# Weepingchestnut/SAVSR

Measured on AMD Instinct MI355X. Metric: HR Mpixels/sec (Vid4-shape x4, 7-frame window), higher is better.
Workload: dtype f32 (bf16x3 split products, fp32 accumulate)

## Files before the change

### savsr_amd/csrc/conv_wy.hip

```cpp
#include "conv_common.hpp"

#include <type_traits>

#ifndef WY_STAMPS
#define WY_STAMPS 0
#endif
#ifndef WY_VALU
#define WY_VALU 6
#endif
#ifndef WY_FAST_EPILOGUE
#define WY_FAST_EPILOGUE 1
#endif
#ifndef WY_BUF
#define WY_BUF 1
#endif

namespace savsr {

namespace wy {
constexpr int TH = 16, TW = 32, NTHR = 512, COT = 64;
[[maybe_unused]] constexpr int IC = TW + 2;
#ifndef WY_ICP
#define WY_ICP 36
#endif
constexpr int ICP = WY_ICP;
constexpr int V_PLANE = 2 * ICP;
constexpr int V_WAVE = 2 * 2 * 2 * V_PLANE;
constexpr int W_HALF = 6 * 2 * 2 * 64;
constexpr int W_PHASE = 2 * W_HALF;
constexpr int EPS = 36;
constexpr int LDS_UNITS = 8 * V_WAVE + 2 * W_HALF;
constexpr size_t LDS_BYTES = 16ull * LDS_UNITS + 4ull * 8 * 32 * EPS;
static_assert(LDS_BYTES <= 160 * 1024, "LDS budget");
}

__device__ __attribute__((aligned(16))) const float g_wy_zero16[4] = {0.f, 0.f, 0.f, 0.f};

#if WY_STAMPS
__device__ long long g_wy_stamps[256 * 8 * 8];
#define WY_KSEC(i) (WY_STAMPS == 2 ? 0 : (i))
#define WY_MARK(i) do { const long long t_now = (long long)__builtin_amdgcn_s_memtime(); wy_sec[i] += t_now - wy_prev; wy_prev = t_now; } while (0)
#if WY_STAMPS == 2
#define WY_EMARK(i) WY_MARK(i)
#endif
#else
#define WY_KSEC(i) (i)
#define WY_MARK(i) do { } while (0)
#endif

typedef float f32x2 __attribute__((ext_vector_type(2)));
typedef __bf16 bf16x2 __attribute__((ext_vector_type(2)));
__device__ __forceinline__ void wy_split_store(const f32x4& v, bf16x4* hi_dst, bf16x4* lo_dst) {
    typedef unsigned u32x2 __attribute__((ext_vector_type(2)));
    const f32x2 a[2] = {{v[0], v[1]}, {v[2], v[3]}};
    u32x2 hi, lo;
#pragma unroll
    for (int p = 0; p < 2; ++p) hi[p] = __builtin_bit_cast(unsigned, __builtin_convertvector(a[p], bf16x2));
    asm("" : "+v"(hi[0]), "+v"(hi[1]));
#pragma unroll
    for (int p = 0; p < 2; ++p) {
        const f32x2 back = {__builtin_bit_cast(float, hi[p] << 16), __builtin_bit_cast(float, hi[p] & 0xffff0000u)};
        const f32x2 rest = {a[p][0] - back[0], a[p][1] - back[1]};
        lo[p] = __builtin_bit_cast(unsigned, __builtin_convertvector(rest, bf16x2));
    }
    *hi_dst = __builtin_bit_cast(bf16x4, hi);
    *lo_dst = __builtin_bit_cast(bf16x4, lo);
}
__device__ __forceinline__ void wy_f16_store(const f32x4& v, bf16x4* hi_dst) {
    f16x4 h;
#pragma unroll
    for (int j = 0; j < 4; ++j) h[j] = (_Float16)v[j];
    *hi_dst = __builtin_bit_cast(bf16x4, h);
}

template <bool FAST, bool F16>
__global__ __launch_bounds__(512) void conv_wy_kernel(const MultiConvParams mp) {
    using namespace wy;
    constexpr int WPH = F16 ? W_PHASE / 2 : W_PHASE, WHF = F16 ? W_HALF / 2 : W_HALF;
    extern __shared__ __attribute__((aligned(16))) unsigned char smem_raw[];
    bf16x8* smem = reinterpret_cast<bf16x8*>(smem_raw);
    const int tid = threadIdx.x, lane = tid & 63, wave = tid >> 6, half = lane >> 5, px = lane & 31;
    const int wave_s = __builtin_amdgcn_readfirstlane(wave);
    const int tiles_per_cob = mp.wy_tiles;
    const int total = mp.nconv * mp.ncob * tiles_per_cob;
    const int H = mp.h, W = mp.w;

    struct TileInfo { int conv, cob, x0, y0, tx, ty, strip; };
    auto decode = [&](int tile) {
        const int cc = (int)((unsigned)tile / (unsigned)tiles_per_cob), rem = tile - cc * tiles_per_cob;
        const bool strip = rem >= mp.wy_full;
        const int tyf = (int)((unsigned)rem / (unsigned)mp.ntx);
        const int l2 = strip ? mp.wy_strip_l2 : 3;
        const int ty = strip ? mp.nty - 1 : tyf;
        const int tx = strip ? (rem - mp.wy_full) << (3 - l2) : rem - tyf * mp.ntx;
        const int wx = tx + (wave_s >> l2);
        TileInfo ti;
        ti.conv = (int)((unsigned)cc / (unsigned)mp.ncob);
        ti.cob = cc - ti.conv * mp.ncob;
        ti.x0 = (wx < mp.ntx ? wx : tx) * TW;
        ti.y0 = wx < mp.ntx ? ty * TH - 2 * ((wave_s >> l2) << l2) : mp.nty * TH;
        ti.tx = tx;
        ti.ty = ty;
        ti.strip = strip ? 1 : 0;
        return ti;
    };

    f32x4 d[2][4], dx;
#if !WY_BUF
    int st_pxb[2], st_pxt;
    constexpr int INVALID = -(1 << 30);
#endif
    const float* st_base = nullptr;
    const bf16x8* st_w = nullptr;
    int st_pix = 0, st_cb = 0, st_src = 0, st_conv = 0, st_row0 = 0;
    const int q4 = lane & 3;
#if WY_BUF
    constexpr unsigned OOB = 0x80000000u;
    unsigned st_vcol[2], st_vtail;
    int st_x0 = 0;
    auto stage_cols = [&]() {
#pragma unroll
        for (int r = 0; r < 2; ++r) {
            const int x = st_x0 - 1 + (lane >> 2) + 16 * r;
            const unsigned v = (unsigned)(x * st_pix + 4 * q4) * 4u;
            st_vcol[r] = (unsigned)x < (unsigned)W ? v : OOB;
        }
        const int x = st_x0 - 1 + 32 + ((lane & 7) >> 2), rr = (lane >> 3) & 3, row = st_row0 + rr;
        const unsigned vt = (unsigned)((rr * W + x) * st_pix + 4 * q4) * 4u;
        const bool okt = (lane < 32) & ((unsigned)x < (unsigned)W) & ((unsigned)row < (unsigned)H);
        st_vtail = okt ? vt : OOB;
    };
#endif
#if WY_BUF
    auto uni = [](int v) { return __builtin_amdgcn_readfirstlane(v); };
    auto uni_ptr = [](const float* q) {
        const unsigned long long a = (unsigned long long)(uintptr_t)q;
        const unsigned lo = (unsigned)__builtin_amdgcn_readfirstlane((int)(unsigned)a), hi = (unsigned)__builtin_amdgcn_readfirstlane((int)(unsigned)(a >> 32));
        return (const float*)(uintptr_t)(((unsigned long long)hi << 32) | lo);
    };
#else
    auto uni = [](int v) { return v; };
    auto uni_ptr = [](const float* q) { return q; };
#endif
    auto stage_begin_tile = [&](const TileInfo& ti) {
        st_conv = ti.conv;
        st_src = 0;
        st_cb = 0;
        st_base = uni_ptr(mp.c[ti.conv].src[0]);
        st_pix = uni(mp.c[ti.conv].src_pix[0]);
        st_w = reinterpret_cast<const bf16x8*>(mp.c[ti.conv].wimg) + (long long)ti.cob * mp.nchunk * WPH;
        st_row0 = uni(ti.y0 + 2 * wave_s - 1);
#if WY_BUF
        st_x0 = ti.x0;
        stage_cols();
#else
#pragma unroll
        for (int r = 0; r < 2; ++r) {
            const int x = ti.x0 - 1 + (lane >> 2) + 16 * r;
            st_pxb[r] = (x >= 0 && x < W) ? st_row0 * W + x : INVALID;
        }
        {
            const int x = ti.x0 - 1 + 32 + ((lane & 7) >> 2), row = st_row0 + ((lane >> 3) & 3);
            st_pxt = (lane < 32 && x >= 0 && x < W && row >= 0 && row < H) ? row * W + x : INVALID;
        }
#endif
    };
    auto stage_advance = [&]() {
        st_cb += 16;
        st_w += WPH;
        if (st_cb >= mp.src_ch) {
            st_cb = 0;
            ++st_src;
            st_base = uni_ptr(mp.c[st_conv].src[st_src]);
#if WY_BUF
            const int pix_new = uni(mp.c[st_conv].src_pix[st_src]);
            if (pix_new != st_pix) { st_pix = pix_new; stage_cols(); }
#else
            st_pix = mp.c[st_conv].src_pix[st_src];
#endif
        }
    };
    int st_tile = blockIdx.x, st_chunk = 0;
    auto stage_next = [&]() -> bool {
        if (st_chunk + 1 < mp.nchunk) { ++st_chunk; stage_advance(); return true; }
        if (st_tile + (int)gridDim.x >= total) return false;
        st_tile += gridDim.x;
        st_chunk = 0;
        stage_begin_tile(decode(st_tile));
        return true;
    };
#if WY_BUF
    typedef unsigned u32x4_t __attribute__((ext_vector_type(4)));
    auto row_rsrc = [&](int i, bool whole) {
        const int off = ((st_row0 + i) * W * st_pix + st_cb) * 4;
        const bool row_ok = whole || (st_row0 + i >= 0 && st_row0 + i < H);
        return __builtin_amdgcn_make_buffer_rsrc((void*)((const char*)st_base + off), (short)0, row_ok ? 0x7fffffff : 0, 0x00020000);
    };
    auto issue_row = [&](int r, int i) {
        d[r][i] = __builtin_bit_cast(f32x4, (u32x4_t)__builtin_amdgcn_raw_buffer_load_b128(row_rsrc(i, false), (int)st_vcol[r], 0, 0));
    };
    auto issue_d = [&](int r) {
#pragma unroll
        for (int i = 0; i < 4; ++i) issue_row(r, i);
    };
    auto issue_dx = [&]() { dx = __builtin_bit_cast(f32x4, (u32x4_t)__builtin_amdgcn_raw_buffer_load_b128(row_rsrc(0, true), (int)st_vtail, 0, 0)); };
#else
    auto load_at = [&](int pixel, bool ok) -> f32x4 {
        const SAVSR_GLOBAL float* src = ok ? (const SAVSR_GLOBAL float*)st_base + (pixel * st_pix + st_cb + 4 * q4)
                                           : (const SAVSR_GLOBAL float*)g_wy_zero16;
        return *(const SAVSR_GLOBAL f32x4*)src;
    };
    auto issue_row = [&](int r, int i) {
        const bool row_ok = st_row0 + i >= 0 && st_row0 + i < H;
        d[r][i] = load_at(st_pxb[r] + i * W, row_ok && st_pxb[r] != INVALID);
    };
    auto issue_d = [&](int r) {
#pragma unroll
        for (int i = 0; i < 4; ++i) issue_row(r, i);
    };
    auto issue_dx = [&]() { dx = load_at(st_pxt, st_pxt != INVALID); };
#endif
    bf16x8* vwave = smem + wave * V_WAVE;
    constexpr int PLANE_B = V_PLANE * 16;
    const unsigned vst0 = (unsigned)(wave * V_WAVE + (q4 >> 1) * ICP + (lane >> 2)) * 16u + (unsigned)(q4 & 1) * 8u;
    const unsigned vst_t = (unsigned)(wave * V_WAVE + (q4 >> 1) * ICP + 32 + ((lane & 7) >> 2)) * 16u + (unsigned)(q4 & 1) * 8u;
    auto vptr = [&](unsigned off) { return reinterpret_cast<bf16x4*>(smem_raw + off); };
    auto vstore = [&](const f32x4& v, unsigned off) {
        if constexpr (F16) wy_f16_store(v, vptr(off));
        else wy_split_store(v, vptr(off), vptr(off + PLANE_B));
    };
    auto store_pair = [&](int r, int hf, const f32x4& va, const f32x4& vb) {
        vstore(va, vst0 + (unsigned)(r * 256 + (hf * 2 + 0) * 2 * PLANE_B));
        vstore(vb, vst0 + (unsigned)(r * 256 + (hf * 2 + 1) * 2 * PLANE_B));
    };
    auto store_one = [&](int r, int hf, int vr, const f32x4& v) {
        vstore(v, vst0 + (unsigned)(r * 256 + (hf * 2 + vr) * 2 * PLANE_B));
    };
    auto store_v0 = [&](int r) { store_one(r, 0, 0, d[r][0] - d[r][2]); };
    auto store_v1 = [&](int r) {
        store_one(r, 0, 1, d[r][1] + d[r][2]);
        const f32x4 v2 = d[r][2] - d[r][1], v3 = d[r][1] - d[r][3];
        d[r][0] = v2;
        d[r][1] = v3;
    };
    auto store_v01 = [&](int r) { store_v0(r); store_v1(r); };
    auto store_v23 = [&](int r) { store_pair(r, 1, d[r][0], d[r][1]); };
    const int grp = (lane >> 3) & 3;
    auto tail_value = [&](int hf) -> f32x4 {
        const int partner = hf == 0 ? (grp == 0 ? lane ^ 16 : lane ^ 24) : (grp == 2 ? lane ^ 24 : lane ^ 16);
        f32x4 o;
#pragma unroll
        for (int j = 0; j < 4; ++j) o[j] = __shfl(dx[j], partner, 64);
        return (hf == 0 && grp == 1) ? dx + o : dx - o;
    };
    auto tail_store = [&](int hf, const f32x4& v) {
        const bool mine = lane < 32 && (hf == 0 ? grp < 2 : (grp == 2 || grp == 1));
        const int vr = hf == 0 ? grp : (grp == 2 ? 0 : 1);
        if (mine) {
            vstore(v, vst_t + (unsigned)((hf * 2 + vr) * 2 * PLANE_B));
        }
    };
    auto store_vt01 = [&]() {
        const f32x4 v01 = tail_value(0), v23 = tail_value(1);
        tail_store(0, v01);
        dx = v23;
    };
    auto store_vt23 = [&]() { tail_store(1, dx); };
    bf16x8* wlds = smem + 8 * V_WAVE;
    [[maybe_unused]] const unsigned lane16 = (unsigned)lane * 16u;
    auto issue_w = [&](int j, int hf) {
        const int piece = F16 ? j * 8 + wave_s : wave_s * 3 + j;
        if (F16 && piece >= 12) return;
        const unsigned dst = __builtin_amdgcn_readfirstlane((unsigned)(uintptr_t)(wlds + hf * W_HALF + piece * (F16 ? 128 : 64)));
        unsigned keep;
#if WY_BUF
        asm volatile("s_mov_b32 %0, m0\n\ts_mov_b32 m0, %3\n\ts_nop 0\n\tglobal_load_lds_dwordx4 %1, %2\n\ts_mov_b32 m0, %0"
                     : "=&s"(keep) : "v"(lane16), "s"(st_w + hf * WHF + piece * 64), "s"(dst) : "memory");
#else
        asm volatile("s_mov_b32 %0, m0\n\ts_mov_b32 m0, %2\n\ts_nop 0\n\tglobal_load_lds_dwordx4 %1, off\n\ts_mov_b32 m0, %0"
                     : "=&s"(keep) : "v"(st_w + hf * WHF + piece * 64 + lane), "s"(dst) : "memory");
#endif
    };

    struct FragA { bf16x8 ah, al; };
    struct FragB { bf16x8 bh, bl; };
    const bf16x8* vrd = vwave + half * ICP + px;
    const bf16x8* wrd = wlds + lane;
    auto load_b = [&](int hf, int s, FragB& fr) {
        const int vr = s / 3, kx = s - 3 * vr;
        fr.bh = vrd[((hf * 2 + vr) * 2 + 0) * V_PLANE + kx];
        if (!F16) fr.bl = vrd[((hf * 2 + vr) * 2 + 1) * V_PLANE + kx];
    };
    auto load_a = [&](int hf, int s, int t, FragA& fr) {
        fr.ah = wrd[hf * W_HALF + ((s * 2 + t) * 2 + 0) * 64];
        if (!F16) fr.al = wrd[hf * W_HALF + ((s * 2 + t) * 2 + 1) * 64];
    };

    int tile = blockIdx.x;
#if WY_STAMPS
    long long wy_sec[8] = {0, 0, 0, 0, 0, 0, 0, 0};
    long long wy_prev = (long long)__builtin_amdgcn_s_memtime();
    const long long wy_t0 = wy_prev;
#endif
    FragA fa[2];
    FragB fb[2];
    if (tile < total) {
        stage_begin_tile(decode(tile));
#pragma unroll
        for (int j = 0; j < 3; ++j) issue_w(j, 0);
        issue_d(0);
        issue_d(1);
        issue_dx();
        store_v01(0);
        store_v01(1);
        store_vt01();
    }
    asm volatile("s_waitcnt vmcnt(0)" ::: "memory");
    __syncthreads();
    if (tile < total) { load_b(0, 0, fb[0]); load_a(0, 0, 0, fa[0]); }

    for (; tile < total; tile += gridDim.x) {
        const TileInfo cur = decode(tile);
        const ConvParams& p = mp.c[cur.conv];
        const int cob = cur.cob, x0 = cur.x0, y0 = cur.y0;
        f32x16 acc[4][2];
#pragma unroll
        for (int pz = 0; pz < 4; ++pz)
#pragma unroll
            for (int t = 0; t < 2; ++t)
#pragma unroll
                for (int i = 0; i < 16; ++i) acc[pz][t][i] = 0.f;
        const bool rows_in = y0 + 2 * wave_s < H;
        for (int chunk = 0; chunk < mp.nchunk; ++chunk) {
            auto phase = [&](auto mm) {
                constexpr bool MM = decltype(mm)::value;
                auto pieces = [&](int hf, int s) {
                    if (hf == 0) {
                        if (s == 0) { issue_w(0, 1); issue_w(1, 1); store_v23(0); }
                        if (s == 1) { issue_w(2, 1); stage_next(); issue_row(0, 0); }
                        if (s == 2) { store_v23(1); issue_row(0, 1); issue_row(0, 2); }
                        if (s == 3) { store_vt23(); issue_row(0, 3); issue_row(1, 0); }
                        if (s == 4) { issue_row(1, 1); issue_row(1, 2); }
                        if (s == 5) issue_row(1, 3);
                    } else {
                        if (s < 3) issue_w(s, 0);
                        if (s == 1) store_v0(0);
                        if (s == 2) store_v1(0);
                        if (s == 3) store_v0(1);
                        if (s == 4) store_v1(1);
                        if (s == 5) store_vt01();
                    }
                };
                auto mma3 = [&](int pz, int t, int sb) {
                    const FragA& a = fa[t];
                    const FragB& b = fb[sb];
                    if (MM && F16) {
                        acc[pz][t] = __builtin_amdgcn_mfma_f32_32x32x16_f16(__builtin_bit_cast(f16x8, a.ah), __builtin_bit_cast(f16x8, b.bh), acc[pz][t], 0, 0, 0);
                    } else if (MM) {
                        acc[pz][t] = __builtin_amdgcn_mfma_f32_32x32x16_bf16(a.al, b.bh, acc[pz][t], 0, 0, 0);
                        acc[pz][t] = __builtin_amdgcn_mfma_f32_32x32x16_bf16(a.ah, b.bl, acc[pz][t], 0, 0, 0);
                        acc[pz][t] = __builtin_amdgcn_mfma_f32_32x32x16_bf16(a.ah, b.bh, acc[pz][t], 0, 0, 0);
                    }
                };
#pragma unroll
                for (int hf = 0; hf < 2; ++hf) {
#pragma unroll
                    for (int s = 0; s < 5; ++s) {
                        const int pz = hf * 2 + s / 3;
                        load_a(hf, s, 1, fa[1]);
                        load_b(hf, s + 1, fb[(s + 1) & 1]);
                        __builtin_amdgcn_sched_barrier(0);
                        mma3(pz, 0, s & 1);
                        pieces(hf, s);
                        load_a(hf, s + 1, 0, fa[0]);
                        mma3(pz, 1, s & 1);
                        if (MM && F16) {
#pragma unroll
                            for (int i = 0; i < 2; ++i) {
                                __builtin_amdgcn_sched_group_barrier(0x008, 1, 0);
                                if (i == 1) __builtin_amdgcn_sched_group_barrier(0x100, 1, 0);
                                __builtin_amdgcn_sched_group_barrier(0x002, 3 * WY_VALU, 0);
                                __builtin_amdgcn_sched_group_barrier(0x200, 2, 0);
                                __builtin_amdgcn_sched_group_barrier(0x010, 1, 0);
                            }
                        } else if (MM) {
#pragma unroll
                            for (int i = 0; i < 6; ++i) {
                                __builtin_amdgcn_sched_group_barrier(0x008, 1, 0);
                                if (i == 3) __builtin_amdgcn_sched_group_barrier(0x100, 2, 0);
                                __builtin_amdgcn_sched_group_barrier(0x002, WY_VALU, 0);
                                __builtin_amdgcn_sched_group_barrier(0x200, 1, 0);
                                if (i == 1 || i == 4) __builtin_amdgcn_sched_group_barrier(0x010, 1, 0);
                            }
                        }
                        __builtin_amdgcn_sched_barrier(0);
                    }
                    {
                        const int pz = hf * 2 + 1;
                        load_a(hf, 5, 1, fa[1]);
                        __builtin_amdgcn_sched_barrier(0);
                        mma3(pz, 0, 1);
                        pieces(hf, 5);
                        if (MM) {
#pragma unroll
                            for (int i = 0; i < (F16 ? 1 : 3); ++i) {
                                __builtin_amdgcn_sched_group_barrier(0x008, 1, 0);
                                __builtin_amdgcn_sched_group_barrier(0x002, 10, 0);
                                __builtin_amdgcn_sched_group_barrier(0x200, 1, 0);
                            }
                        }
                        __builtin_amdgcn_sched_barrier(0);
                        WY_MARK(WY_KSEC(hf * 3 + 0));
                        if (hf == 0) asm volatile("s_waitcnt vmcnt(8)" ::: "memory");
                        else asm volatile("s_waitcnt vmcnt(0)" ::: "memory");
                        __syncthreads();
                        WY_MARK(WY_KSEC(hf * 3 + 1));
                        load_b(hf ^ 1, 0, fb[0]);
                        load_a(hf ^ 1, 0, 0, fa[0]);
                        __builtin_amdgcn_sched_barrier(0);
                        mma3(pz, 1, 1);
                        if (hf == 0) issue_dx();
                        __builtin_amdgcn_sched_barrier(0);
                    }
                    WY_MARK(WY_KSEC(hf * 3 + 2));
                }
            };
            auto phase_dead = [&]() {
#pragma unroll
                for (int j = 0; j < 3; ++j) issue_w(j, 1);
                stage_next();
                asm volatile("s_waitcnt vmcnt(0)" ::: "memory");
                __syncthreads();
#pragma unroll
                for (int j = 0; j < 3; ++j) issue_w(j, 0);
                asm volatile("s_waitcnt vmcnt(0)" ::: "memory");
                __syncthreads();
            };
            auto next_tile_rows_in = [&]() {
                if (tile + (int)gridDim.x >= total) return false;
                return decode(tile + (int)gridDim.x).y0 + 2 * wave_s < H;
            };
            if (rows_in) phase(std::true_type{});
            else if (chunk + 1 == mp.nchunk && next_tile_rows_in()) phase(std::false_type{});
            else phase_dead();
        }

        const float* e_bias = p.bias;
        const float* e_mul = p.mul_px;
        const float* e_r1 = p.res1;
        const float* e_r2 = p.res2;
        float* e_out = p.out;
        float* e_pool = p.pool;
        int e_act = p.act, e_opix = p.out_pix, e_r1pix = p.res1_pix, e_r2pix = p.res2_pix;
        float e_slope = p.slope, e_r2s = p.res2_scale;
        asm volatile("" : "+s"(e_bias), "+s"(e_mul), "+s"(e_r1), "+s"(e_r2), "+s"(e_out), "+s"(e_pool));
        asm volatile("" : "+s"(e_act), "+s"(e_opix), "+s"(e_r1pix), "+s"(e_r2pix), "+s"(e_slope), "+s"(e_r2s));
        const bool act_as_max = e_act == SAVSR_ACT_NONE || e_act == SAVSR_ACT_RELU || (e_act == SAVSR_ACT_LRELU && e_slope >= 0.f && e_slope <= 1.f);
        const float slope_eff = e_act == SAVSR_ACT_NONE ? 1.f : (e_act == SAVSR_ACT_RELU ? 0.f : e_slope);
        float* ep_base = reinterpret_cast<float*>(smem + LDS_UNITS);
        float* ep = ep_base + wave * (32 * EPS);
        const int c4 = lane & 7;
        const bool x_inside = x0 + TW <= W;
        const float* zero16 = (const float*)g_wy_zero16;
        const float* b_base = e_bias ? e_bias : zero16;
        const unsigned b_off = e_bias ? 4u * (unsigned)(cob * COT + 4 * c4) : 0u, b_step = e_bias ? 128u : 0u;
        f32x4 bias4[2];
#pragma unroll
        for (int t = 0; t < 2; ++t) bias4[t] = ldg4(b_base, b_off + (unsigned)t * b_step);
        const float* r1_base = e_r1 ? e_r1 : zero16;
        constexpr int RR = 2;
        f32x4 rr[RR][4];
        auto load_r1 = [&](int r, int t, f32x4 (&dst)[4]) {
            const int y = y0 + 2 * wave_s + r;
            const int co = cob * COT + 32 * t + 4 * c4;
            const unsigned off0 = 4u * (unsigned)((y * W + x0 + (lane >> 3)) * e_r1pix + co), ustride = 32u * (unsigned)e_r1pix;
            const bool row_ok = e_r1 && y < H;
#pragma unroll
            for (int i = 0; i < 4; ++i) {
                const bool ok = row_ok && (x_inside || x0 + (lane >> 3) + 8 * i < W);
                dst[i] = ldg4(r1_base, ok ? off0 + (unsigned)i * ustride : 0u);
            }
        };
#pragma unroll
        for (int gi = 0; gi < RR; ++gi) load_r1(gi / 2, gi % 2, rr[gi]);
        __builtin_amdgcn_sched_barrier(0);
#pragma unroll
        for (int t = 0; t < 2; ++t)
#pragma unroll
            for (int i = 0; i < 16; ++i) {
                const float m1 = acc[1][t][i], m2 = acc[2][t][i];
                acc[0][t][i] = (acc[0][t][i] + m1) + m2;
                acc[3][t][i] = (m1 - m2) - acc[3][t][i];
            }
        f32x4 psum[2][2];
#ifdef WY_EMARK
        asm volatile("" :: "v"(acc[0][0][0]), "v"(acc[3][1][15]));
        WY_EMARK(1);
#endif
#pragma unroll
        for (int r = 0; r < 2; ++r) {
            const int y = y0 + 2 * wave_s + r;
            const int pbase = y * W + x0 + (lane >> 3);
#pragma unroll
            for (int t = 0; t < 2; ++t) {
                psum[r][t] = f32x4{0.f, 0.f, 0.f, 0.f};
                const int gi = r * 2 + t;
                if (y >= H) {
                    asm volatile("" :: "v"(bias4[t]), "v"(rr[gi % RR][0]), "v"(rr[gi % RR][1]), "v"(rr[gi % RR][2]), "v"(rr[gi % RR][3]));
                    if (gi + RR < 4) load_r1((gi + RR) / 2, (gi + RR) % 2, rr[gi % RR]);
                    continue;
                }
                const f32x16& a = r == 0 ? acc[0][t] : acc[3][t];
#pragma unroll
                for (int g = 0; g < 4; ++g) {
                    const f32x4 v = {a[4 * g], a[4 * g + 1], a[4 * g + 2], a[4 * g + 3]};
                    *reinterpret_cast<f32x4*>(ep + px * EPS + 8 * g + 4 * half) = v;
                }
                const int co = cob * COT + 32 * t + 4 * c4;
                const f32x4 b4 = bias4[t];
                const unsigned ooff0 = 4u * (unsigned)(pbase * e_opix + co), ostride = 32u * (unsigned)e_opix;
                f32x4 ps = {0.f, 0.f, 0.f, 0.f};
#pragma unroll
                for (int ih = 0; ih < 2; ++ih) {
                    const int p0 = pbase + 16 * ih;
                    const bool ok0 = x_inside || x0 + (lane >> 3) + 16 * ih < W, ok1 = x_inside || x0 + (lane >> 3) + 16 * ih + 8 < W;
                    f32x4 v[2];
#pragma unroll
                    for (int i = 0; i < 2; ++i) {
                        const f32x4 a4 = *reinterpret_cast<const f32x4*>(ep + ((lane >> 3) + 16 * ih + 8 * i) * EPS + 4 * c4);
                        v[i] = a4 + b4;
                    }
                    if constexpr (FAST) {
#pragma unroll
                        for (int i = 0; i < 2; ++i) {
                            const f32x4 sv = v[i] * slope_eff;
#pragma unroll
                            for (int q = 0; q < 4; ++q) v[i][q] = vmax_raw(v[i][q], sv[q]);
                        }
                    } else if (e_act == SAVSR_ACT_NONE) {
                    } else if (act_as_max) {
#pragma unroll
                        for (int i = 0; i < 2; ++i) {
                            const f32x4 sv = v[i] * slope_eff;
#pragma unroll
                            for (int q = 0; q < 4; ++q) v[i][q] = vmax_raw(v[i][q], sv[q]);
                        }
                    } else if (e_act == SAVSR_ACT_LRELU) {
#pragma unroll
                        for (int i = 0; i < 2; ++i)
#pragma unroll
                            for (int q = 0; q < 4; ++q) v[i][q] = v[i][q] > 0.f ? v[i][q] : v[i][q] * e_slope;
                    } else if (e_act == SAVSR_ACT_SIGMOID) {
#pragma unroll
                        for (int i = 0; i < 2; ++i)
#pragma unroll
                            for (int q = 0; q < 4; ++q) v[i][q] = sigmoidf_(v[i][q]);
                    }
                    if (!FAST && e_mul) {
                        const float m0 = ok0 ? ldg1(e_mul, (unsigned)p0) : 0.f, m1 = ok1 ? ldg1(e_mul, (unsigned)(p0 + 8)) : 0.f;
#pragma unroll
                        for (int q = 0; q < 4; ++q) { v[0][q] *= m0; v[1][q] *= m1; }
                    }
                    v[0] += rr[gi % RR][2 * ih];
                    v[1] += rr[gi % RR][2 * ih + 1];
                    if (!FAST && e_r2) {
                        f32x4 ra = {0.f, 0.f, 0.f, 0.f}, rb = {0.f, 0.f, 0.f, 0.f};
                        if (ok0) ra = ldg4(e_r2, 4u * (unsigned)(p0 * e_r2pix + co));
                        if (ok1) rb = ldg4(e_r2, 4u * (unsigned)((p0 + 8) * e_r2pix + co));
#pragma unroll
                        for (int q = 0; q < 4; ++q) { v[0][q] += e_r2s * ra[q]; v[1][q] += e_r2s * rb[q]; }
                    }
#pragma unroll
                    for (int i = 0; i < 2; ++i) {
                        if (i == 0 ? ok0 : ok1) {
                            stg4(e_out, ooff0 + (unsigned)(2 * ih + i) * ostride, v[i]);
                            if (e_pool) ps += v[i];
                        }
                    }
                }
                psum[r][t] = ps;
#ifdef WY_EMARK
                WY_EMARK(2 + gi);
#endif
                if (gi + RR < 4) load_r1((gi + RR) / 2, (gi + RR) % 2, rr[gi % RR]);
            }
        }
        if (e_pool) {
#pragma unroll
            for (int r = 0; r < 2; ++r)
#pragma unroll
                for (int t = 0; t < 2; ++t)
#pragma unroll
                    for (int o = 8; o < 64; o <<= 1) {
                        psum[r][t][0] += __shfl_xor(psum[r][t][0], o, 64); psum[r][t][1] += __shfl_xor(psum[r][t][1], o, 64);
                        psum[r][t][2] += __shfl_xor(psum[r][t][2], o, 64); psum[r][t][3] += __shfl_xor(psum[r][t][3], o, 64);
                    }
            __syncthreads();
            float* pl_ = ep_base;
            if (lane < 8)
#pragma unroll
                for (int r = 0; r < 2; ++r)
#pragma unroll
                    for (int t = 0; t < 2; ++t) *reinterpret_cast<f32x4*>(pl_ + (wave * 2 + r) * COT + 32 * t + 4 * lane) = psum[r][t];
            __syncthreads();
            const TileInfo pt = decode(tile);
            const int l2p = pt.strip ? mp.wy_strip_l2 : 2;
            if (tid < (8 >> l2p) * COT) {
                const int sg = tid / COT, ch = tid - sg * COT;
                float sacc = 0.f;
#pragma unroll
                for (int k = 0; k < 8; ++k)
                    if (k < (2 << l2p)) sacc += pl_[(((sg << l2p) * 2) + k) * COT + ch];
                const int band = pt.ty * 2 + (pt.strip ? 0 : sg), ptx = pt.tx + (pt.strip ? sg : 0);
                if (band * 8 < H && ptx < mp.ntx) stg1(e_pool, (unsigned)((band * mp.ntx + ptx) * p.pool_stride + cob * COT + ch), sacc);
            }
            __syncthreads();
        }
        WY_MARK(6);
    }
#if WY_STAMPS
    wy_sec[7] = (long long)__builtin_amdgcn_s_memtime() - wy_t0;
    if (lane == 0 && blockIdx.x < 256)
        for (int i = 0; i < 8; ++i) g_wy_stamps[(blockIdx.x * 8 + wave) * 8 + i] = wy_sec[i];
#endif
    asm volatile("s_waitcnt vmcnt(0)" ::: "memory");
}

int launch_conv_wy(const MultiConvParams& mp, hipStream_t st, bool f16) {
    if (int rc = conv_wy_prepare_device()) return rc;
    const int total = mp.nconv * mp.ncob * mp.wy_tiles;
    const int grid = total < CONV_PERSISTENT_BLOCKS ? total : CONV_PERSISTENT_BLOCKS;
    bool fast = WY_FAST_EPILOGUE != 0;
    for (int i = 0; i < mp.nconv && fast; ++i) {
        const ConvParams& c = mp.c[i];
        const bool as_max = c.act == SAVSR_ACT_NONE || c.act == SAVSR_ACT_RELU || (c.act == SAVSR_ACT_LRELU && c.slope >= 0.f && c.slope <= 1.f);
        fast = as_max && !c.mul_px && !c.res2;
    }
    if (f16) {
        if (fast) hipLaunchKernelGGL((conv_wy_kernel<true, true>), dim3(grid), dim3(wy::NTHR), wy::LDS_BYTES, st, mp);
        else hipLaunchKernelGGL((conv_wy_kernel<false, true>), dim3(grid), dim3(wy::NTHR), wy::LDS_BYTES, st, mp);
    } else if (fast) hipLaunchKernelGGL((conv_wy_kernel<true, false>), dim3(grid), dim3(wy::NTHR), wy::LDS_BYTES, st, mp);
    else hipLaunchKernelGGL((conv_wy_kernel<false, false>), dim3(grid), dim3(wy::NTHR), wy::LDS_BYTES, st, mp);
    return check_launch("conv_wy_kernel");
}
int conv_wy_prepare_device() {
    if (int rc = ensure_dynamic_lds(reinterpret_cast<const void*>(&conv_wy_kernel<true, false>), (int)wy::LDS_BYTES, "conv_wy")) return rc;
    if (int rc = ensure_dynamic_lds(reinterpret_cast<const void*>(&conv_wy_kernel<false, false>), (int)wy::LDS_BYTES, "conv_wy")) return rc;
    if (int rc = ensure_dynamic_lds(reinterpret_cast<const void*>(&conv_wy_kernel<true, true>), (int)wy::LDS_BYTES, "conv_wy")) return rc;
    return ensure_dynamic_lds(reinterpret_cast<const void*>(&conv_wy_kernel<false, true>), (int)wy::LDS_BYTES, "conv_wy");
}

}

using namespace savsr;

#if WY_STAMPS
extern "C" int savsr_debug_read_wy_stamps(long long* host) {
    return (int)hipMemcpyFromSymbol(host, HIP_SYMBOL(g_wy_stamps), sizeof(long long) * 256 * 8 * 8);
}
#endif

extern "C" int64_t savsr_conv_wy_packed_elems(int cout, int cin) {
    if (cout <= 0 || cout % 64 || cin <= 0 || cin % 16) return -1;
    return (int64_t)(cout / 64) * (cin / 16) * 12 * 16 * 64;
}
extern "C" int64_t savsr_conv_wy_pack_index(int cout, int cin, int co, int ci, int pos, int kx) {
    const int64_t nchunk = cin / 16;
    const int cob = co / 64, col = co % 64, t = col / 32, row = col % 32;
    const int chunk = ci / 16, cl = ci % 16, kh = cl / 8, j = cl % 8;
    const int hf = pos / 2, vr = pos % 2, s = vr * 3 + kx;
    const int64_t group = ((((int64_t)(cob * nchunk + chunk) * 2 + hf) * 6 + s) * 2 + t);
    return group * 512 + (kh * 32 + row) * 8 + j;
}
```

Baseline: 141.0.

## Micro-optimize WY conv epilogue with packed math, MFMA zeroing and DPP pooling reduction

Zeroes the accumulators with zero-input MFMA instructions instead of many VALU moves. Rewrites the Winograd output transform and the leaky-relu scaling as packed two-wide float ops (pk_fma/pk_mul). Replaces the shuffle-based pooling reduction with DPP row shifts plus permlane16/32 swaps, so the four partial sums are folded together and written by more lanes at once. The goal is fewer VALU and LDS-shuffle instructions in the epilogue, at the cost of relying on gfx950-specific permlane builtins and a more intricate lane mapping that has to reproduce the old pooling layout exactly.

```diff
diff --git a/savsr_amd/csrc/conv_wy.hip b/savsr_amd/csrc/conv_wy.hip
--- a/savsr_amd/csrc/conv_wy.hip
+++ b/savsr_amd/csrc/conv_wy.hip
@@ -66,6 +66,12 @@
     *hi_dst = __builtin_bit_cast(bf16x4, hi);
     *lo_dst = __builtin_bit_cast(bf16x4, lo);
 }
+__device__ __forceinline__ f32x4 wy_scale4(const f32x4& v, float s) {
+    f32x2 lo = f32x2{v[0], v[1]} * s, hi = f32x2{v[2], v[3]} * s;
+    asm("" : "+v"(lo), "+v"(hi));
+    return f32x4{lo[0], lo[1], hi[0], hi[1]};
+}
+__device__ __forceinline__ f32x2 wy_sub2(const f32x2& a, const f32x2& b, const f32x2& neg1) { return __builtin_elementwise_fma(b, neg1, a); }
 __device__ __forceinline__ void wy_f16_store(const f32x4& v, bf16x4* hi_dst) {
     f16x4 h;
 #pragma unroll
@@ -324,12 +330,21 @@
         const ConvParams& p = mp.c[cur.conv];
         const int cob = cur.cob, x0 = cur.x0, y0 = cur.y0;
         f32x16 acc[4][2];
-#pragma unroll
-        for (int pz = 0; pz < 4; ++pz)
-#pragma unroll
-            for (int t = 0; t < 2; ++t)
-#pragma unroll
-                for (int i = 0; i < 16; ++i) acc[pz][t][i] = 0.f;
+        {
+            typedef unsigned u32x4_z __attribute__((ext_vector_type(4)));
+            unsigned zs = 0u;
+            asm volatile("" : "+s"(zs));
+            u32x4_z zbits = {zs, zs, zs, zs};
+            const f32x16 c0 = {0.f, 0.f, 0.f, 0.f, 0.f, 0.f, 0.f, 0.f, 0.f, 0.f, 0.f, 0.f, 0.f, 0.f, 0.f, 0.f};
+#pragma unroll
+            for (int pz = 0; pz < 4; ++pz)
+#pragma unroll
+                for (int t = 0; t < 2; ++t) {
+                    asm volatile("" : "+v"(zbits));
+                    const bf16x8 z = __builtin_bit_cast(bf16x8, zbits);
+                    acc[pz][t] = __builtin_amdgcn_mfma_f32_32x32x16_bf16(z, z, c0, 0, 0, 0);
+                }
+        }
         const bool rows_in = y0 + 2 * wave_s < H;
         for (int chunk = 0; chunk < mp.nchunk; ++chunk) {
             auto phase = [&](auto mm) {
@@ -484,13 +499,17 @@
 #pragma unroll
         for (int gi = 0; gi < RR; ++gi) load_r1(gi / 2, gi % 2, rr[gi]);
         __builtin_amdgcn_sched_barrier(0);
+        f32x2 neg1 = {-1.f, -1.f};
+        asm volatile("" : "+v"(neg1));
 #pragma unroll
         for (int t = 0; t < 2; ++t)
 #pragma unroll
-            for (int i = 0; i < 16; ++i) {
-                const float m1 = acc[1][t][i], m2 = acc[2][t][i];
-                acc[0][t][i] = (acc[0][t][i] + m1) + m2;
-                acc[3][t][i] = (m1 - m2) - acc[3][t][i];
+            for (int i = 0; i < 16; i += 2) {
+                const f32x2 a0 = {acc[0][t][i], acc[0][t][i + 1]}, m1 = {acc[1][t][i], acc[1][t][i + 1]};
+                const f32x2 m2 = {acc[2][t][i], acc[2][t][i + 1]}, a3 = {acc[3][t][i], acc[3][t][i + 1]};
+                const f32x2 o0 = (a0 + m1) + m2, o1 = wy_sub2(wy_sub2(m1, m2, neg1), a3, neg1);
+                acc[0][t][i] = o0[0]; acc[0][t][i + 1] = o0[1];
+                acc[3][t][i] = o1[0]; acc[3][t][i + 1] = o1[1];
             }
         f32x4 psum[2][2];
 #ifdef WY_EMARK
@@ -533,7 +552,7 @@
                     if constexpr (FAST) {
 #pragma unroll
                         for (int i = 0; i < 2; ++i) {
-                            const f32x4 sv = v[i] * slope_eff;
+                            const f32x4 sv = wy_scale4(v[i], slope_eff);
 #pragma unroll
                             for (int q = 0; q < 4; ++q) v[i][q] = vmax_raw(v[i][q], sv[q]);
                         }
@@ -541,7 +560,7 @@
                     } else if (act_as_max) {
 #pragma unroll
                         for (int i = 0; i < 2; ++i) {
-                            const f32x4 sv = v[i] * slope_eff;
+                            const f32x4 sv = wy_scale4(v[i], slope_eff);
 #pragma unroll
                             for (int q = 0; q < 4; ++q) v[i][q] = vmax_raw(v[i][q], sv[q]);
                         }
@@ -586,22 +605,28 @@
             }
         }
         if (e_pool) {
-#pragma unroll
-            for (int r = 0; r < 2; ++r)
-#pragma unroll
-                for (int t = 0; t < 2; ++t)
-#pragma unroll
-                    for (int o = 8; o < 64; o <<= 1) {
-                        psum[r][t][0] += __shfl_xor(psum[r][t][0], o, 64); psum[r][t][1] += __shfl_xor(psum[r][t][1], o, 64);
-                        psum[r][t][2] += __shfl_xor(psum[r][t][2], o, 64); psum[r][t][3] += __shfl_xor(psum[r][t][3], o, 64);
-                    }
+            auto f2u = [](float x) { return __builtin_bit_cast(unsigned, x); };
+            auto u2f = [](unsigned x) { return __builtin_bit_cast(float, x); };
+            f32x4 pred;
+#pragma unroll
+            for (int q = 0; q < 4; ++q) {
+                float h[2];
+#pragma unroll
+                for (int r = 0; r < 2; ++r) {
+#pragma unroll
+                    for (int t = 0; t < 2; ++t)
+                        psum[r][t][q] += u2f((unsigned)__builtin_amdgcn_update_dpp(0, (int)f2u(psum[r][t][q]), 0x128, 0xf, 0xf, false));
+                    const auto sw = __builtin_amdgcn_permlane16_swap(f2u(psum[r][0][q]), f2u(psum[r][1][q]), false, false);
+                    h[r] = u2f(sw[0]) + u2f(sw[1]);
+                }
+                const auto sw = __builtin_amdgcn_permlane32_swap(f2u(h[0]), f2u(h[1]), false, false);
+                pred[q] = u2f(sw[0]) + u2f(sw[1]);
+            }
             __syncthreads();
             float* pl_ = ep_base;
-            if (lane < 8)
-#pragma unroll
-                for (int r = 0; r < 2; ++r)
-#pragma unroll
-                    for (int t = 0; t < 2; ++t) *reinterpret_cast<f32x4*>(pl_ + (wave * 2 + r) * COT + 32 * t + 4 * lane) = psum[r][t];
+            int pl_lane = lane;
+            asm volatile("" : "+v"(pl_lane));
+            if ((pl_lane & 8) == 0) *reinterpret_cast<f32x4*>(pl_ + wave * 2 * COT + 32 * (pl_lane >> 4) + 4 * (pl_lane & 7)) = pred;
             __syncthreads();
             const TileInfo pt = decode(tile);
             const int l2p = pt.strip ? mp.wy_strip_l2 : 2;
```

New measurement: 142.0 (median of 6 runs). Within noise of the previous version (+0.7%).
